# wolfcanli/ORB_SLAM2_Modification_with-point-and-line-feature

Measured on AMD Instinct MI355X. Metric: frames/sec (extract+match+pose) at 640x480; ATE RMSE vs ref, higher is better.
Workload: dtype u8

## Files before the change

### orb_slam2_modification_with-point-and-line-feature_amd/csrc/orb_extract.hip

```cpp
#include <hip/hip_runtime.h>
#include <algorithm>
#include <stdint.h>

#include <cstdlib>

#include "orb_geom.h"
#include "orbpl_math.h"
#include "orb_kernels.h"
#include "orbpl_runtime.h"

namespace orbpl {

#include "orb_pattern.inc"
__constant__ int c_pattern[1024];
__constant__ float4 c_pattern_f[256];

__device__ __forceinline__ int reflect101_dev(int p, int len) {
  if (p < 0) p = -p;
  if (p >= len) p = 2 * len - 2 - p;
  return p;
}

__host__ __device__ constexpr int fast_pstride(int win_w) { return (win_w + 7) & ~7; }
__host__ __device__ constexpr int fast_wave_words(int win_w, int win_h) {
  return win_h * (fast_pstride(win_w) / 2) + 4 * win_h;
}

typedef short fshort2 __attribute__((ext_vector_type(2)));
typedef unsigned short fushort2 __attribute__((ext_vector_type(2)));
typedef uint32_t fuint3 __attribute__((ext_vector_type(3)));
typedef fuint3 fuint3_a4 __attribute__((aligned(4)));

__device__ __forceinline__ uint32_t umul24(uint32_t a, uint32_t b) {
  return (uint32_t)(uint16_t)a * (uint32_t)(uint16_t)b;
}
template <uint32_t D>
__device__ __forceinline__ uint32_t div_c16(uint32_t i) {
  return umul24(i, (65536u + D - 1) / D) >> 16;
}
__device__ __forceinline__ int imul24(int a, int b) {
  return (int)(int16_t)a * (int)(int16_t)b;
}
__device__ __forceinline__ uint32_t ld_dw(const uint32_t* base, uint32_t dw) {
  return *reinterpret_cast<const uint32_t*>(reinterpret_cast<const char*>(base) + (dw << 2));
}
__device__ __forceinline__ void ld_dw3(const uint32_t* base, uint32_t dw, uint32_t* a, uint32_t* b,
                                       uint32_t* c) {
  const char* p = reinterpret_cast<const char*>(base) + (dw << 2);
  *a = *reinterpret_cast<const uint32_t*>(p);
  *b = *reinterpret_cast<const uint32_t*>(p + 4);
  *c = *reinterpret_cast<const uint32_t*>(p + 8);
}
__device__ __forceinline__ uint32_t ld_b4(const uint8_t* base, uint32_t off) {
  return *reinterpret_cast<const uint32_t*>(base + off);
}
__device__ __forceinline__ void st_b4(uint8_t* base, uint32_t off, uint32_t v) {
  *reinterpret_cast<uint32_t*>(base + off) = v;
}

__device__ __forceinline__ fshort2 as_s2(uint32_t v) { return __builtin_bit_cast(fshort2, v); }
__device__ __forceinline__ fushort2 as_u2(uint32_t v) { return __builtin_bit_cast(fushort2, v); }
__device__ __forceinline__ fshort2 pmin(fshort2 a, fshort2 b) { return __builtin_elementwise_min(a, b); }
__device__ __forceinline__ fshort2 pmax(fshort2 a, fshort2 b) { return __builtin_elementwise_max(a, b); }
__device__ __forceinline__ fushort2 pmaxu(fushort2 a, fushort2 b) { return __builtin_elementwise_max(a, b); }
__device__ __forceinline__ fushort2 pminu(fushort2 a, fushort2 b) { return __builtin_elementwise_min(a, b); }

__device__ __forceinline__ uint32_t ring_pair(const uint2* R, int dy, int dx) {
  const uint32_t j = (uint32_t)(3 + dx);
  return __builtin_amdgcn_perm(R[3 + dy].y, R[3 + dy].x, j | (0x0cu << 8) | ((j + 1) << 16) | (0x0cu << 24));
}

template <bool kMax>
__device__ __forceinline__ void fast_windows(const fushort2* p, fushort2* W) {
  auto op = [](fushort2 a, fushort2 b) { return kMax ? pmaxu(a, b) : pminu(a, b); };
  fushort2 s[2][4], pr[2][4];
#pragma unroll
  for (int h = 0; h < 2; h++) {
    const fushort2* d = p + 8 * h;
    const fushort2 q12 = op(d[1], d[2]), q34 = op(d[3], d[4]), q56 = op(d[5], d[6]);
    s[h][3] = d[7];
    s[h][2] = op(q56, d[7]);
    s[h][1] = op(q34, s[h][2]);
    s[h][0] = op(q12, s[h][1]);
    pr[h][0] = d[0];
    pr[h][1] = op(d[0], q12);
    pr[h][2] = op(pr[h][1], q34);
    pr[h][3] = op(pr[h][2], q56);
  }
#pragma unroll
  for (int i = 0; i < 4; i++) {
    W[i] = op(s[0][i], pr[1][i]);
    W[i + 4] = op(s[1][i], pr[0][i]);
  }
}

__device__ __forceinline__ fshort2 fast_m2_regs(const uint2* R) {
  const fushort2 v = as_u2(ring_pair(R, 0, 0));
  fushort2 p[16];
  p[0] = as_u2(ring_pair(R, 3, 0));
  p[1] = as_u2(ring_pair(R, 3, 1));
  p[2] = as_u2(ring_pair(R, 2, 2));
  p[3] = as_u2(ring_pair(R, 1, 3));
  p[4] = as_u2(ring_pair(R, 0, 3));
  p[5] = as_u2(ring_pair(R, -1, 3));
// ... 1148 lines not shown
        }
      }
    }
    __syncthreads();
    cur = nxt;
    size = newSize;
    if (size >= N || size == prevSize) {
      finish = true;
    } else if (!phase2 && size + nexp * 3 > N) {
      phase2 = true;
    }
  }
  lap(1);
  for (int i = t; i < size; i += NT) S.child[i] = 0;
  __syncthreads();
  for (int k = t; k < total; k += NT) {
    uint32_t c = K[k];
    int key = (cand_s(c) << 20) | (kMaxCandPerLevel - k);
    atomicMax(&S.child[kn_get(k)], key);
  }
  __syncthreads();
  const int cap = L.kp_cap;
  for (int i = t; i < size && i < cap; i += NT) {
    int k = kMaxCandPerLevel - (S.child[i] & kMaxCandPerLevel);
    out_list[i] = K[k];
  }
  if (t == 0) {
    if (size > cap) atomicOr(err_flag, 4);
    *out_count = size < cap ? size : cap;
  }
  lap(3);
  ot[5] = total;
  ot[6] = size;
  if (stamp)
    for (int k = 0; k < 8; k++) g_oct_prof[8 * level + k] = ot[k];
}

__device__ long long g_od_prof[8];

constexpr int kIcR = 15;
constexpr int kIcRowDw = 9;
constexpr int kIcDw = (2 * kIcR + 1) * kIcRowDw;
constexpr int kIcLoads = (kIcDw + 63) / 64;
constexpr int kBriefR = 18;
constexpr int kBriefRows = 2 * kBriefR + 1;
constexpr int kBriefRowDw = 10;
constexpr int kBriefDw = kBriefRows * kBriefRowDw;
constexpr int kBriefLoads = (kBriefDw + 63) / 64;

#ifndef ORBPL_OD_MINW
#define ORBPL_OD_MINW 1
#endif

__device__ __forceinline__ void ic_dword(uint32_t px, int u0, int um, int* s0, int* s1) {
  const int lo = min(max(-um - u0, 0), 4), hi = min(max(um - u0 + 1, 0), 4);
  const uint32_t m = hi > lo ? (0xFFFFFFFFu >> (8 * (4 - (hi - lo)))) << (8 * lo) : 0u;
  const uint32_t pm = px & m;
  const int a = (int)__builtin_amdgcn_udot4(pm, 0x01010101u, 0u, false);
  const int b = (int)__builtin_amdgcn_udot4(pm, 0x03020100u, 0u, false);
  *s0 += a;
  *s1 += imul24(u0, a) + b;
}
__global__ void __launch_bounds__(256, ORBPL_OD_MINW) k_orient_desc(const uint8_t* __restrict__ pyr,
                                                     const uint8_t* __restrict__ blur,
                                                     const OrbGeom* __restrict__ g,
                                                     const uint32_t* __restrict__ kp_list,
                                                     const int* __restrict__ kp_count,
                                                     orbpl_keypoint_dev* __restrict__ out_kps,
                                                     uint8_t* __restrict__ out_desc,
                                                     int kp_pitch, int* __restrict__ out_n,
                                                      int slot0, int slot1, int write_n) {
  __shared__ uint32_t s_patch[4][kBriefDw];
  const int wave = threadIdx.x >> 6, lane = threadIdx.x & 63;
  int bx, f;
  xcd_block(&bx, &f);
  const int slot = slot0 + bx * 4 + wave;
  if (slot >= slot1) return;
  const bool stamp = g_oct_prof_on && f == 0 && slot == 0 && lane == 0;
  long long dt[6] = {0, 0, 0, 0, 0, 0};
  long long d0 = stamp ? (long long)wall_clock64() : 0;
  auto lap = [&](int k) {
    if (stamp) {
      const long long d1 = (long long)wall_clock64();
      dt[k] = d1 - d0;
      d0 = d1;
    }
  };
  int level = 0;
  while (level + 1 < g->nlevels && slot >= g->lv[level + 1].kp_base) level++;
  const LevelGeom& L = g->lv[level];
  const int idx = slot - L.kp_base;
  const int* cnts = kp_count + (long long)f * g->nlevels;
  int offset = 0, total = 0;
  for (int l = 0; l < g->nlevels; l++) {
    int c = cnts[l];
    if (l < level) offset += c;
    total += c;
  }
  if (write_n && slot == slot0 && lane == 0) out_n[f] = total < kp_pitch ? total : kp_pitch;
  if (idx >= cnts[level]) return;
  const int opos = offset + idx;
  if (opos >= kp_pitch) return;
  lap(0);
  const uint32_t c = kp_list[(long long)f * g->kp_cap_total + slot];
  const int kx = cand_x(c) + kMinBorder, ky = cand_y(c) + kMinBorder;
  if (stamp) (void)__builtin_amdgcn_readfirstlane(kx);
  lap(1);
  const uint8_t* irow0 = pyr + (long long)f * g->pyr_bytes + content_off(L, kx - kIcR, ky - kIcR);
  const int io = (int)(reinterpret_cast<uintptr_t>(irow0) & 3);
  const uint32_t* irow = reinterpret_cast<const uint32_t*>(irow0 - io);
  const int ipdw = L.pitch >> 2;
  uint32_t iv[kIcLoads];
#pragma unroll
  for (int j = 0; j < kIcLoads; j++) {
    const int i = lane + 64 * j;
// ... 44 lines not shown
  cr_cos_sin(angle * factorPI, &a, &b);
  if (stamp) (void)__builtin_amdgcn_readfirstlane(__float_as_int(a + b));
  lap(3);
  uint32_t* patch = s_patch[wave];
#pragma unroll
  for (int j = 0; j < kBriefLoads; j++) {
    const int i = lane + 64 * j;
    if (i < kBriefDw) patch[i] = pv[j];
  }
  __builtin_amdgcn_wave_barrier();
  const uint8_t* bimg = reinterpret_cast<const uint8_t*>(patch) + kBriefR * 4 * kBriefRowDw +
                        (bx0 & 3) + kBriefR;
  const int step = 4 * kBriefRowDw;
  uint64_t words[4];
#pragma unroll
  for (int r = 0; r < 4; r++) {
    const int tst = r * 64 + lane;
    const int* p = &c_pattern[4 * tst];
    const float x1 = (float)p[0], y1 = (float)p[1], x2 = (float)p[2], y2 = (float)p[3];
    const int v1 = bimg[cv_round(x1 * b + y1 * a) * step + cv_round(x1 * a - y1 * b)];
    const int v2 = bimg[cv_round(x2 * b + y2 * a) * step + cv_round(x2 * a - y2 * b)];
    words[r] = __ballot(v1 < v2);
  }
  lap(4);
  uint8_t* d = out_desc + ((long long)f * kp_pitch + opos) * 32;
  if (lane < 4) {
    uint64_t w = lane == 0 ? words[0] : lane == 1 ? words[1] : lane == 2 ? words[2] : words[3];
    reinterpret_cast<uint64_t*>(d)[lane] = w;
  }
  if (lane == 0) {
    orbpl_keypoint_dev kp;
    float sx = (float)kx, sy = (float)ky;
    if (level != 0) {
      sx = sx * L.scale;
      sy = sy * L.scale;
    }
    kp.x = sx;
    kp.y = sy;
    kp.size = (float)L.scaled_patch;
    kp.angle = angle;
    kp.response = (float)cand_s(c);
    kp.octave = level;
    kp.class_id = -1;
    out_kps[(long long)f * kp_pitch + opos] = kp;
  }
  lap(5);
  if (stamp)
    for (int k = 0; k < 6; k++) g_od_prof[k] = dt[k];
}

#ifndef ORBPL_OD_PAIR
#define ORBPL_OD_PAIR 1
#endif
constexpr int kIcLoads2 = (kIcDw + 31) / 32;
constexpr int kBriefLoads2 = (kBriefDw + 31) / 32;
__global__ void __launch_bounds__(256, ORBPL_OD_MINW) k_orient_desc2(const uint8_t* __restrict__ pyr,
                                                      const uint8_t* __restrict__ blur,
                                                      const OrbGeom* __restrict__ g,
                                                      const uint32_t* __restrict__ kp_list,
                                                      const int* __restrict__ kp_count,
                                                      orbpl_keypoint_dev* __restrict__ out_kps,
                                                      uint8_t* __restrict__ out_desc,
                                                      int kp_pitch, int* __restrict__ out_n,
                                                      int slot0, int slot1, int write_n) {
  __shared__ uint32_t s_patch[8][kBriefDw];
  const int wave = threadIdx.x >> 6, lane = threadIdx.x & 63;
  const int half = lane >> 5, l32 = lane & 31;
  int bx, f;
  xcd_block(&bx, &f);
  const int slot = slot0 + bx * 8 + wave * 2 + half;
  const int nlev = g->nlevels;
  bool act = slot < slot1;
  int level = 0;
  if (act)
    while (level + 1 < nlev && slot >= g->lv[level + 1].kp_base) level++;
  const LevelGeom& L = g->lv[level];
  const int idx = slot - L.kp_base;
  const int* cnts = kp_count + (long long)f * nlev;
  int offset = 0, total = 0, mine = 0;
  for (int l = 0; l < nlev; l++) {
    const int c = cnts[l];
    if (l < level) offset += c;
    if (l == level) mine = c;
    total += c;
  }
  if (write_n && slot == slot0 && l32 == 0) out_n[f] = total < kp_pitch ? total : kp_pitch;
  act = act && idx < mine && offset + idx < kp_pitch;
  if (!__any(act)) return;
  const int opos = offset + idx;
  const uint32_t c = act ? kp_list[(long long)f * g->kp_cap_total + slot] : 0u;
  const int kx = act ? cand_x(c) + kMinBorder : kIcR + kBriefR,
            ky = act ? cand_y(c) + kMinBorder : kIcR + kBriefR;
  const uint32_t* fpyr = reinterpret_cast<const uint32_t*>(pyr + (long long)f * g->pyr_bytes);
  const int ioff = (int)content_off(L, kx - kIcR, ky - kIcR);
  const int io = ioff & 3;
  const uint32_t ibase = (uint32_t)ioff >> 2;
  const uint32_t ipdw = (uint32_t)L.pitch >> 2;
  uint32_t iv[kIcLoads2];
#pragma unroll
  for (int j = 0; j < kIcLoads2; j++) {
    const uint32_t i = (uint32_t)l32 + 32u * j;
    const uint32_t r = div_c16<kIcRowDw>(i), q = i - umul24(r, kIcRowDw);
    iv[j] = (act && i < (uint32_t)kIcDw) ? ld_dw(fpyr, ibase + umul24(r, ipdw) + q) : 0u;
  }
  const int bx0 = kx - kBriefR;
  const uint32_t* fblur = reinterpret_cast<const uint32_t*>(blur + (long long)f * g->blur_bytes);
  const uint32_t pdw = (uint32_t)L.bpitch >> 2;
  const uint32_t pbase =
      (uint32_t)((L.boff + (long long)(ky - kBriefR) * L.bpitch + (bx0 & ~3)) >> 2);
  uint32_t pv[kBriefLoads2];
#pragma unroll
  for (int j = 0; j < kBriefLoads2; j++) {
    const uint32_t i = (uint32_t)l32 + 32u * j;
    const uint32_t r = div_c16<kBriefRowDw>(i), q = i - umul24(r, kBriefRowDw);
    pv[j] = (act && i < (uint32_t)kBriefDw) ? ld_dw(fblur, pbase + umul24(r, pdw) + q) : 0u;
  }
  int m01 = 0, m10 = 0;
#pragma unroll
  for (int j = 0; j < kIcLoads2; j++) {
    const int i = l32 + 32 * j;
    const int r = (int)div_c16<kIcRowDw>((uint32_t)i), q = i - (int)umul24((uint32_t)r, kIcRowDw);
    const int v = r - kIcR;
    const int um = i < kIcDw ? g->umax[v < 0 ? -v : v] : -1;
    int s0 = 0;
    ic_dword(iv[j], 4 * q - io - kIcR, um, &s0, &m10);
    m01 += imul24(v, s0);
  }
#pragma unroll
  for (int o = 16; o >= 1; o >>= 1) {
    m10 += __shfl_xor(m10, o, 64);
    m01 += __shfl_xor(m01, o, 64);
  }
  const float angle = fast_atan2_deg((float)m01, (float)m10);
  const float factorPI = (float)(3.14159265358979323846 / 180.f);
  float a, b;
  cr_cos_sin(angle * factorPI, &a, &b);
  uint32_t* patch = s_patch[wave * 2 + half];
#pragma unroll
  for (int j = 0; j < kBriefLoads2; j++) {
    const int i = l32 + 32 * j;
    if (i < kBriefDw) patch[i] = pv[j];
  }
  __builtin_amdgcn_wave_barrier();
  const uint8_t* bimg = reinterpret_cast<const uint8_t*>(patch) + kBriefR * 4 * kBriefRowDw +
                        (bx0 & 3) + kBriefR;
  const int step = 4 * kBriefRowDw;
  uint32_t words[8];
#pragma unroll
  for (int r = 0; r < 8; r++) {
    const float4 P = c_pattern_f[r * 32 + l32];
    const float x1 = P.x, y1 = P.y, x2 = P.z, y2 = P.w;
    const float fs = (float)step;
    const int v1 = bimg[(int)(__builtin_rintf(x1 * b + y1 * a) * fs + __builtin_rintf(x1 * a - y1 * b))];
    const int v2 = bimg[(int)(__builtin_rintf(x2 * b + y2 * a) * fs + __builtin_rintf(x2 * a - y2 * b))];
    words[r] = (uint32_t)(__ballot(v1 < v2) >> (32 * half));
  }
  if (!act) return;
  uint8_t* d = out_desc + ((long long)f * kp_pitch + opos) * 32;
  if (l32 < 8) {
    uint32_t w = words[0];
#pragma unroll
    for (int r = 1; r < 8; r++) w = l32 == r ? words[r] : w;
    reinterpret_cast<uint32_t*>(d)[l32] = w;
  }
  if (l32 == 0) {
    orbpl_keypoint_dev kp;
    float sx = (float)kx, sy = (float)ky;
    if (level != 0) {
      sx = sx * L.scale;
      sy = sy * L.scale;
    }
    kp.x = sx;
    kp.y = sy;
    kp.size = (float)L.scaled_patch;
    kp.angle = angle;
    kp.response = (float)cand_s(c);
    kp.octave = level;
    kp.class_id = -1;
    out_kps[(long long)f * kp_pitch + opos] = kp;
  }
}

hipError_t upload_pattern(hipStream_t s) {
  static float pf[1024];
  static const bool filled = [] {
    for (int i = 0; i < 1024; i++) pf[i] = (float)bit_pattern_31_[i];
    return true;
  }();
  (void)filled;
  const hipError_t e = hipMemcpyToSymbolAsync(HIP_SYMBOL(c_pattern), bit_pattern_31_,
                                              sizeof(bit_pattern_31_), 0, hipMemcpyHostToDevice, s);
  if (e != hipSuccess) return e;
  return hipMemcpyToSymbolAsync(HIP_SYMBOL(c_pattern_f), pf, sizeof(pf), 0, hipMemcpyHostToDevice, s);
}
// ... 14 lines not shown
                    hipStream_t s) {
  hipLaunchKernelGGL(k_pyramid, dim3(nbands, batch), dim3(kPyrThreads), 0, s, img, stride,
                     frame_pitch, pyr, blur, dg, rs, bands, prof, l0, l1);
}

void launch_fast(const OrbGeom& hg, const OrbGeom* dg, const CellGeom* cells, const uint8_t* pyr,
                 uint32_t* cell_cands, int* cell_counts, int ini_th, int min_th, int batch,
                 int l0, int l1, hipStream_t s) {
  const size_t smem = 4 * 4 * (size_t)fast_wave_words(hg.fast_win_w, hg.fast_win_h);
  const int c0 = hg.lv[l0].cell_base;
  const int c1 = l1 < hg.nlevels ? hg.lv[l1].cell_base : hg.ncells_total;
  if (c1 <= c0) return;
  hipLaunchKernelGGL(k_fast_cells, dim3((c1 - c0 + 3) / 4, batch), dim3(256), smem, s, pyr, dg,
                     cells, cell_cands, cell_counts, ini_th, min_th, c0, c1);
}

void launch_octree(const OrbGeom& hg, const OrbGeom* dg, const uint32_t* cell_cands,
                   const int* cell_counts, uint32_t* kcand, int* knode, uint32_t* kp_list,
                   int* kp_count, int* err_flag, int batch, int l0, int l1, int wave_from,
                   hipStream_t s) {
  set_smem_attr((const void*)k_octree<1024, 256>, sizeof(OctShared<1024>));
  int cap = 0;
  for (int l = 0; l < hg.nlevels; l++) cap = std::max(cap, hg.lv[l].kp_cap);
  if (once_per_device((const void*)&g_oct_prof_on)) {
    const int on = getenv("ORBPL_OCT_PROFILE") ? 1 : 0;
    (void)hipMemcpyToSymbolAsync(HIP_SYMBOL(g_oct_prof_on), &on, sizeof(int), 0,
                                 hipMemcpyHostToDevice, s);
  }
  const bool one_wave = l0 >= (wave_from >= 0 ? wave_from : kOctWaveFrom);
#define ORBPL_OCT_LAUNCH(CAP)                                                                   \
  if (one_wave)                                                                                 \
    hipLaunchKernelGGL((k_octree<CAP, 64>), dim3(l1 - l0, batch), dim3(64),                    \
                       sizeof(OctShared<CAP, 2048>), s, dg, cell_cands, cell_counts, kcand,     \
                       knode,                                                                   \
                       kp_list, kp_count, err_flag, l0);                                        \
  else                                                                                          \
    hipLaunchKernelGGL((k_octree<CAP, 256>), dim3(l1 - l0, batch), dim3(256),                  \
                       sizeof(OctShared<CAP>), s, dg, cell_cands, cell_counts, kcand, knode,    \
                       kp_list, kp_count, err_flag, l0);
  if (cap <= 256) {
    ORBPL_OCT_LAUNCH(256)
  } else if (cap <= 512) {
    ORBPL_OCT_LAUNCH(512)
  } else {
    if (one_wave) set_smem_attr((const void*)k_octree<1024, 64>, sizeof(OctShared<1024, 2048>));
    ORBPL_OCT_LAUNCH(1024)
  }
#undef ORBPL_OCT_LAUNCH
}

void launch_orient_desc(const OrbGeom& hg, const OrbGeom* dg, const uint8_t* pyr,
                        const uint8_t* blur, const uint32_t* kp_list, const int* kp_count,
                        orbpl_keypoint_dev* out_kps, uint8_t* out_desc, int kp_pitch, int* out_n,
                        int batch, int l0, int l1, hipStream_t s) {
  const int s0 = hg.lv[l0].kp_base;
  const int s1 = l1 < hg.nlevels ? hg.lv[l1].kp_base : hg.kp_cap_total;
  const int wn = l1 == hg.nlevels ? 1 : 0;
  if (s1 <= s0) return;
  static const char* pe = getenv("ORBPL_OD_PAIR");
  static const bool pair = (pe ? atoi(pe) != 0 : ORBPL_OD_PAIR) && !getenv("ORBPL_OCT_PROFILE");
  if (pair)
    hipLaunchKernelGGL(k_orient_desc2, dim3((s1 - s0 + 7) / 8, batch), dim3(256), 0, s, pyr, blur,
                       dg, kp_list, kp_count, out_kps, out_desc, kp_pitch, out_n, s0, s1, wn);
  else
    hipLaunchKernelGGL(k_orient_desc, dim3((s1 - s0 + 3) / 4, batch), dim3(256), 0, s, pyr, blur,
                       dg, kp_list, kp_count, out_kps, out_desc, kp_pitch, out_n, s0, s1, wn);
}

}
```

### orb_slam2_modification_with-point-and-line-feature_amd/csrc/orb_geom.cpp

```cpp
#include <algorithm>
#include <cmath>
#include <vector>

#include "../../include/orbpl.h"
#include "orb_kernels.h"

namespace orbpl {

static int round_up(int v, int a) { return (v + a - 1) / a * a; }

int build_orb_geometry(int nfeatures, float scale_factor, int nlevels, int W, int H,
                       OrbHostGeom* out, const char** err) {
  *err = nullptr;
  if (nlevels < 1 || nlevels > kMaxLevels) { *err = "nlevels out of range [1,16]"; return ORBPL_ERR_ARG; }
  if (nfeatures < 1) { *err = "nfeatures must be >= 1"; return ORBPL_ERR_ARG; }
  if (!(scale_factor > 1.0f)) { *err = "scale_factor must be > 1"; return ORBPL_ERR_ARG; }
  if (W > 4000 || H > 4000) { *err = "image larger than 4000 px is not supported"; return ORBPL_ERR_ARG; }
  OrbHostGeom& G = *out;
  OrbGeom& g = G.g;
  g = OrbGeom{};
  g.nlevels = nlevels;
  g.W = W;
  g.H = H;
  const double sf = (double)scale_factor;
  G.scale.assign(nlevels, 1.0f);
  G.sigma2.assign(nlevels, 1.0f);
  for (int i = 1; i < nlevels; i++) {
    G.scale[i] = (float)(G.scale[i - 1] * sf);
    G.sigma2[i] = G.scale[i] * G.scale[i];
  }
  G.inv_scale.resize(nlevels);
  G.inv_sigma2.resize(nlevels);
  for (int i = 0; i < nlevels; i++) {
    G.inv_scale[i] = 1.0f / G.scale[i];
    G.inv_sigma2[i] = 1.0f / G.sigma2[i];
  }
  std::vector<int> nfeat(nlevels);
  {
    const float factor = (float)(1.0f / sf);
    float nd = nfeatures * (1 - factor) / (1 - (float)std::pow((double)factor, (double)nlevels));
    int sum = 0;
    for (int l = 0; l < nlevels - 1; l++) {
      nfeat[l] = (int)std::rint(nd);
      sum += nfeat[l];
      nd *= factor;
    }
    nfeat[nlevels - 1] = std::max(nfeatures - sum, 0);
  }
  {
    const int HP = 15;
    int v, v0;
    const int vmax = (int)std::floor(HP * std::sqrt(2.f) / 2 + 1);
    const int vmin = (int)std::ceil(HP * std::sqrt(2.f) / 2);
    const double hp2 = HP * HP;
    for (v = 0; v <= vmax; ++v) g.umax[v] = (int)std::rint(std::sqrt(hp2 - v * v));
    for (v = HP, v0 = 0; v >= vmin; --v) {
      while (g.umax[v0] == g.umax[v0 + 1]) ++v0;
      g.umax[v] = v0;
      ++v0;
    }
  }
  long long off = 0, boff = 0;
  int cell_total = 0, kp_total = 0;
  int max_slots = 1;
  G.cells.clear();
  G.rs.clear();
  std::vector<std::vector<CellGeom>> lvl_cells(nlevels);
  for (int l = 0; l < nlevels; l++) {
    LevelGeom& L = g.lv[l];
    L.w = (int)std::rint((float)W * G.inv_scale[l]);
    L.h = (int)std::rint((float)H * G.inv_scale[l]);
    if (L.w < 20 || L.h < 20) {
      *err = "a pyramid level is smaller than 20 px (image too small for nlevels/scale)";
      return ORBPL_ERR_ARG;
    }
    L.pw = L.w + 2 * kEdge;
    L.ph = L.h + 2 * kEdge;
    L.pitch = round_up(kLead + L.pw, 16);
    L.pyr_off = off;
    off += (long long)round_up(L.pitch * L.ph, 256);
    L.bpitch = round_up(L.w, 16);
    L.boff = boff;
    boff += (long long)round_up(L.bpitch * L.h, 256);
    L.scale = G.scale[l];
    L.nfeat = nfeat[l];
    L.scaled_patch = (int)(31 * G.scale[l]);
    const int minB = kMinBorder;
    const int maxBX = L.w - kEdge + 3, maxBY = L.h - kEdge + 3;
    L.max_border_x = maxBX;
    L.max_border_y = maxBY;
    const float width = (float)(maxBX - minB), height = (float)(maxBY - minB);
    const int nCols = (int)(width / 30.f), nRows = (int)(height / 30.f);
    L.ncols = nCols;
    L.nrows = nRows;
    L.wcell = nCols > 0 ? (int)std::ceil(width / nCols) : 0;
    L.hcell = nRows > 0 ? (int)std::ceil(height / nRows) : 0;
    L.ncells = nCols * nRows;
    L.cell_base = cell_total;
    for (int i = 0; i < nRows; i++) {
      const float iniY = (float)(minB + i * L.hcell);
      float maxY = iniY + L.hcell + 6;
      for (int j = 0; j < nCols; j++) {
        CellGeom c{};
        c.level = (int16_t)l;
        const float iniX = (float)(minB + j * L.wcell);
        float maxX = iniX + L.wcell + 6;
        bool skip = (iniY >= maxBY - 3) || (iniX >= maxBX - 6);
        if (!skip) {
          float my = maxY > maxBY ? (float)maxBY : maxY;
          float mx = maxX > maxBX ? (float)maxBX : maxX;
          c.x0 = (int16_t)iniX;
          c.y0 = (int16_t)iniY;
          c.x1 = (int16_t)mx;
// ... 111 lines not shown
```

### orb_slam2_modification_with-point-and-line-feature_amd/csrc/orb_geom.h

```cpp
#pragma once
#include <stdint.h>

namespace orbpl {

constexpr int kMaxLevels = 16;
constexpr int kEdge = 19;
constexpr int kMinBorder = 16;
constexpr int kLead = 13;
constexpr int kContent0 = kLead + 19;
constexpr int kOctMaxList = 1024;
constexpr int kMaxCandPerLevel = (1 << 20) - 1;

struct LevelGeom {
  int w, h;
  int pw, ph;
  int pitch;
  int pad0;
  long long pyr_off;
  float scale;
  int nfeat;
  int ncols, nrows;
  int wcell, hcell;
  int cell_base;
  int ncells;
  int max_border_x, max_border_y;
  int n_ini;
  float hx;
  int kp_cap;
  int kp_base;
  int cand_base;
  int cand_cap;
  int rs_off;
  int xmax;
  int scaled_patch;
  int pad2, pad3;
  int bpitch;
  int pad1;
  long long boff;
};

struct CellGeom {
  int16_t x0, y0, x1, y1;
  int16_t level, pad;
};

struct OrbGeom {
  int nlevels;
  int W, H;
  int ncells_total;
  int kp_cap_total;
  int cand_cap_total;
  int cell_slots;
  int fast_win_w;
  int fast_win_h;
  long long pyr_bytes;
  long long blur_bytes;
  int umax[16];
  LevelGeom lv[kMaxLevels];
};

#ifndef ORBPL_PYR_THREADS
#define ORBPL_PYR_THREADS 256
#endif
constexpr int kPyrThreads = ORBPL_PYR_THREADS;
constexpr int kPyrMaxBands = 8;
struct PyrBand {
  int na[kMaxLevels], nb[kMaxLevels];
  int oa[kMaxLevels], ob[kMaxLevels];
};
__host__ __device__ inline int pyr_band_base(int B) { return B - 1; }

__host__ __device__ inline long long content_off(const LevelGeom& L, int x, int y) {
  return L.pyr_off + (long long)(y + kEdge) * L.pitch + kContent0 + x;
}
__host__ __device__ inline long long padded_off(const LevelGeom& L, int px, int py) {
  return L.pyr_off + (long long)py * L.pitch + kLead + px;
}

__host__ __device__ inline uint32_t pack_cand(int x, int y, int s) {
  return (uint32_t)x | ((uint32_t)y << 12) | ((uint32_t)s << 24);
}
__host__ __device__ inline int cand_x(uint32_t c) { return (int)(c & 0xFFF); }
__host__ __device__ inline int cand_y(uint32_t c) { return (int)((c >> 12) & 0xFFF); }
__host__ __device__ inline int cand_s(uint32_t c) { return (int)(c >> 24); }

}
```

### orb_slam2_modification_with-point-and-line-feature_amd/csrc/orb_kernels.h

```cpp
#pragma once
#include <hip/hip_runtime.h>
#include <stdint.h>

#include <vector>

#include "orb_geom.h"

namespace orbpl {

struct orbpl_keypoint_dev {
  float x, y, size, angle, response;
  int octave, class_id;
};

hipError_t upload_pattern(hipStream_t s);
int read_octree_profile(long long* out128);
int read_od_profile(long long* out8);

void launch_pyramid(const OrbGeom& hg, const OrbGeom* dg, const uint8_t* img, int stride,
                    long long frame_pitch, uint8_t* pyr, uint8_t* blur, const int* rs,
                    const PyrBand* bands, int nbands, int batch, long long* prof, int l0, int l1,
                    hipStream_t s);
void launch_fast(const OrbGeom& hg, const OrbGeom* dg, const CellGeom* cells, const uint8_t* pyr,
                 uint32_t* cell_cands, int* cell_counts, int ini_th, int min_th, int batch,
                 int l0, int l1, hipStream_t s);
void launch_octree(const OrbGeom& hg, const OrbGeom* dg, const uint32_t* cell_cands,
                   const int* cell_counts, uint32_t* kcand, int* knode, uint32_t* kp_list,
                   int* kp_count, int* err_flag, int batch, int l0, int l1, int wave_from,
                   hipStream_t s);
void launch_orient_desc(const OrbGeom& hg, const OrbGeom* dg, const uint8_t* pyr,
                        const uint8_t* blur, const uint32_t* kp_list, const int* kp_count,
                        orbpl_keypoint_dev* out_kps, uint8_t* out_desc, int kp_pitch, int* out_n,
                        int batch, int l0, int l1, hipStream_t s);

struct OrbHostGeom {
  OrbGeom g;
  std::vector<CellGeom> cells;
  std::vector<int> rs;
  std::vector<PyrBand> bands;
  std::vector<float> scale, inv_scale, sigma2, inv_sigma2;
};
int build_orb_geometry(int nfeatures, float scale_factor, int nlevels, int W, int H,
                       OrbHostGeom* out, const char** err);

}
```

### orb_slam2_modification_with-point-and-line-feature_amd/csrc/orbpl_runtime.cpp

```cpp
#include <dirent.h>
#include <hip/hip_runtime.h>

#include <cstdio>
#include <cstdlib>
#include <cstring>
#include <unistd.h>
#include <mutex>
#include <map>
#include <set>
#include <cctype>
#include <string>
#include <utility>
#include <vector>

#include "../../include/orbpl.h"
#include "orb_kernels.h"
#include "host_stage.h"
#include "orbpl_runtime.h"

namespace orbpl {

int g_hw_queues = 4;
int g_runtime_started = 0;
int g_queues_set_by_lib = 0;
// ... 64 lines not shown
  static std::set<std::pair<const void*, int>> seen;
  int dev = 0;
  (void)hipGetDevice(&dev);
  std::lock_guard<std::mutex> lk(mu);
  return seen.insert({key, dev}).second;
}

void set_smem_attr(const void* fn, size_t bytes) {
  if (once_per_device(fn))
    (void)hipFuncSetAttribute(fn, hipFuncAttributeMaxDynamicSharedMemorySize, (int)bytes);
}

int device_cu_count() {
  static std::mutex mu;
  static std::map<int, int> cus;
  int dev = 0;
  (void)hipGetDevice(&dev);
  std::lock_guard<std::mutex> lk(mu);
  auto it = cus.find(dev);
  if (it != cus.end()) return it->second;
  int n = 0;
  if (hipDeviceGetAttribute(&n, hipDeviceAttributeMultiprocessorCount, dev) != hipSuccess || n <= 0)
    n = 256;
  cus[dev] = n;
  return n;
}

}

using namespace orbpl;

struct orbx_ctx {
  orbpl_orb_params params{};
  int device = 0;
  int max_batch = 0;
  OrbHostGeom hg;
  hipStream_t stream = nullptr;
  hipEvent_t ev[6] = {};
  hipStream_t fstream = nullptr;
  hipEvent_t ev_group[kMaxLevels] = {};
  hipEvent_t ev_fjoin = nullptr;
  hipEvent_t ev_kern[kKernelBrackets] = {};
  int ngroups = 1;
  int group_end[kMaxLevels] = {};
  bool timed = false;
  OrbGeom* d_geom = nullptr;
  CellGeom* d_cells = nullptr;
  int* d_rs = nullptr;
  PyrBand* d_bands = nullptr;
  long long* d_pyr_prof = nullptr;
  int pyr_bands = 0;
  int group_bands[kFastGroups] = {0, 0, 0, 0};
  int oct_wave_from = -1;
  uint8_t* d_in = nullptr;
  uint8_t* d_pyr = nullptr;
  uint8_t* d_blur = nullptr;
  uint32_t* d_cell_cands = nullptr;
  int* d_cell_counts = nullptr;
  uint32_t* d_kcand = nullptr;
  int* d_knode = nullptr;
  uint32_t* d_kp_list = nullptr;
  int* d_kp_count = nullptr;
  orbpl_keypoint_dev* d_out_kps = nullptr;
  uint8_t* d_out_desc = nullptr;
  int* d_out_n = nullptr;
  int* d_err = nullptr;
  int last_batch = 0;
};

extern "C" {

const char* orbpl_last_error(void) { return orbpl::g_last_error.c_str(); }

const char* orbpl_version(void) { return "orbpl gfx950 r4"; }

int orbpl_hw_queue_state(int* queues, int* runtime_started, int* set_by_library,
                         int* lsd_split_1024) {
  if (queues) *queues = orbpl::g_hw_queues;
  if (runtime_started) *runtime_started = orbpl::g_runtime_started;
  if (set_by_library) *set_by_library = orbpl::g_queues_set_by_lib;
  if (lsd_split_1024) *lsd_split_1024 = orbpl::lsd_split_decision(1024) ? 1 : 0;
  return ORBPL_OK;
}

int orbpl_device_count(int* n) {
  if (!n) return arg_fail("n is NULL");
  int c = 0;
  hipError_t e = hipGetDeviceCount(&c);
  if (e != hipSuccess) {
    *n = 0;
    hip_fail(e, "hipGetDeviceCount", __LINE__);
    return ORBPL_ERR_NODEVICE;
  }
  *n = c;
  return c > 0 ? ORBPL_OK : ORBPL_ERR_NODEVICE;
}

int orbpl_dev_malloc(int device, int64_t bytes, void** out) {
  if (!out || bytes < 0) return arg_fail("bad argument");
  HIP_CHECK(hipSetDevice(device));
  HIP_CHECK(hipMalloc(out, (size_t)(bytes > 0 ? bytes : 1)));
  return ORBPL_OK;
}

int orbpl_dev_free(int device, void* ptr) {
  HIP_CHECK(hipSetDevice(device));
// ... 140 lines not shown
    if (c->ngroups > 1) {
      CK(hipStreamCreateWithFlags(&c->fstream, hipStreamNonBlocking));
      for (int i = 0; i < c->ngroups; i++)
        CK(hipEventCreateWithFlags(&c->ev_group[i], hipEventDisableTiming));
      CK(hipEventCreateWithFlags(&c->ev_fjoin, hipEventDisableTiming));
    }
  }
  const size_t B = (size_t)max_batch;
  CK(hipMalloc(&c->d_geom, sizeof(OrbGeom)));
  CK(hipMalloc(&c->d_cells, sizeof(CellGeom) * std::max<size_t>(1, c->hg.cells.size())));
  CK(hipMalloc(&c->d_rs, sizeof(int) * c->hg.rs.size()));
  CK(hipMalloc(&c->d_bands, sizeof(PyrBand) * c->hg.bands.size()));
  CK(hipMalloc(&c->d_in, B * (size_t)width * height));
  CK(hipMalloc(&c->d_pyr, B * (size_t)g.pyr_bytes));
  CK(hipMalloc(&c->d_blur, B * (size_t)g.blur_bytes));
  CK(hipMalloc(&c->d_cell_cands, B * (size_t)std::max(1, g.ncells_total) * g.cell_slots * 4));
  CK(hipMalloc(&c->d_cell_counts, B * (size_t)std::max(1, g.ncells_total) * 4));
  CK(hipMalloc(&c->d_kcand, B * (size_t)std::max(1, g.cand_cap_total) * 4));
  CK(hipMalloc(&c->d_knode, B * (size_t)std::max(1, g.cand_cap_total) * 4));
  CK(hipMalloc(&c->d_kp_list, B * (size_t)g.kp_cap_total * 4));
  CK(hipMalloc(&c->d_kp_count, B * (size_t)g.nlevels * 4));
  CK(hipMalloc(&c->d_out_kps, B * (size_t)g.kp_cap_total * sizeof(orbpl_keypoint_dev)));
  CK(hipMalloc(&c->d_out_desc, B * (size_t)g.kp_cap_total * 32));
  CK(hipMalloc(&c->d_out_n, B * 4));
  CK(hipMalloc(&c->d_err, 4));
  CK(hipMemsetAsync(c->d_err, 0, 4, c->stream));
  CK(hipMemsetAsync(c->d_pyr, 0, B * (size_t)g.pyr_bytes, c->stream));
  CK(hipMemsetAsync(c->d_blur, 0, B * (size_t)g.blur_bytes, c->stream));
  CK(hipMemcpyAsync(c->d_geom, &g, sizeof(OrbGeom), hipMemcpyHostToDevice, c->stream));
  if (!c->hg.cells.empty())
    CK(hipMemcpyAsync(c->d_cells, c->hg.cells.data(), sizeof(CellGeom) * c->hg.cells.size(),
                      hipMemcpyHostToDevice, c->stream));
  CK(hipMemcpyAsync(c->d_rs, c->hg.rs.data(), sizeof(int) * c->hg.rs.size(), hipMemcpyHostToDevice,
                    c->stream));
  CK(hipMemcpyAsync(c->d_bands, c->hg.bands.data(), sizeof(PyrBand) * c->hg.bands.size(),
                    hipMemcpyHostToDevice, c->stream));
  if (const char* e = getenv("ORBPL_PYR_BANDS")) {
    const int b = atoi(e);
    if (b == 1 || b == 2 || b == 4 || b == 8) c->pyr_bands = b;
  }
  if (const char* e = getenv("ORBPL_PYR_GROUP_BANDS")) {
    int gi = 0;
    for (const char* q = e; *q && gi < kFastGroups;) {
      if (!isdigit((unsigned char)*q)) {
        q++;
        continue;
      }
      const int b = atoi(q);
      while (isdigit((unsigned char)*q)) q++;
      c->group_bands[gi++] = (b == 1 || b == 2 || b == 4 || b == 8) ? b : 0;
    }
  }
  if (const char* e = getenv("ORBPL_OCT_WAVE_FROM")) c->oct_wave_from = std::max(0, atoi(e));
  if (getenv("ORBPL_PYR_PROFILE")) {
    CK(hipMalloc(&c->d_pyr_prof, 8 * (1 + 4 * kMaxLevels)));
    CK(hipMemsetAsync(c->d_pyr_prof, 0, 8 * (1 + 4 * kMaxLevels), c->stream));
  }
  CK(upload_pattern(c->stream));
  CK(hipStreamSynchronize(c->stream));
#undef CK
  *out = c;
  return ORBPL_OK;
}

int orbx_debug_pyr_profile(orbx_ctx* c, long long* out, int cap, int* n) {
  if (!c || !out || !n) return arg_fail("bad argument");
  if (!c->d_pyr_prof) return arg_fail("ORBPL_PYR_PROFILE was not set when the context was created");
  HIP_CHECK(hipStreamSynchronize(c->stream));
  const int L = c->hg.g.nlevels;
  std::vector<long long> p(1 + 4 * kMaxLevels);
  HIP_CHECK(hipMemcpy(p.data(), c->d_pyr_prof, p.size() * 8, hipMemcpyDeviceToHost));
  *n = std::min(cap, 4 * L);
  for (int i = 0; i < *n; i++) out[i] = (p[i + 1] - p[i]) * 10;
  return ORBPL_OK;
}

int orbx_debug_octree_profile(orbx_ctx* c, long long* out128) {
  if (!c || !out128) return arg_fail("bad argument");
  HIP_CHECK(hipStreamSynchronize(c->stream));
  if (read_octree_profile(out128)) return arg_fail("octree profile unavailable");
  for (int l = 0; l < 16; l++)
    for (int k : {0, 1, 2, 3}) out128[8 * l + k] *= 10;
  long long od[6];
  if (read_od_profile(od) == 0)
    for (int k = 0; k < 6; k++) out128[120 + k] = od[k] * 10;
  return ORBPL_OK;
}

int orbx_destroy(orbx_ctx* c) {
  free_ctx(c);
  return ORBPL_OK;
}

int orbx_get_scale_info(const orbx_ctx* c, int* nlevels, float* scale, float* inv_scale,
                        float* sigma2, float* inv_sigma2) {
  if (!c) return arg_fail("NULL ctx");
  const int n = c->hg.g.nlevels;
  if (nlevels) *nlevels = n;
  for (int i = 0; i < n; i++) {
    if (scale) scale[i] = c->hg.scale[i];
    if (inv_scale) inv_scale[i] = c->hg.inv_scale[i];
    if (sigma2) sigma2[i] = c->hg.sigma2[i];
    if (inv_sigma2) inv_sigma2[i] = c->hg.inv_sigma2[i];
  }
  return ORBPL_OK;
}
// ... 32 lines not shown
namespace orbpl {
hipStream_t orbx_stream(orbx_ctx* c) { return c->stream; }

constexpr int kLevelPipeMinBatch = 64;

int orbx_run(orbx_ctx* c, const uint8_t* d_imgs, int batch, int stride, long long frame_pitch,
             orbpl_keypoint_dev* d_kps, uint8_t* d_desc, int kp_pitch, int* d_n,
             hipEvent_t* ext_events, hipEvent_t* ext_kernels) {
  const OrbGeom& g = c->hg.g;
  hipStream_t s = c->stream;
  c->timed = ext_events == nullptr;
  hipEvent_t* ev = ext_events ? ext_events : c->ev;
  hipEvent_t* evk = ext_kernels ? ext_kernels : (ext_events ? nullptr : c->ev_kern);
  HIP_CHECK(hipEventRecord(ev[0], s));
  int nb = c->pyr_bands;
  if (!nb) {
    nb = 1;
    while (nb < kPyrMaxBands && nb * batch < 1024) nb *= 2;
  }
  auto bracket = [&](int kind, int gi, int end, hipStream_t st) -> hipError_t {
    return evk ? hipEventRecord(evk[2 * (kind * kFastGroups + gi) + end], st) : hipSuccess;
  };
  const bool pipe = c->ngroups > 1 && batch >= kLevelPipeMinBatch;
  const int ngroups = pipe ? c->ngroups : 1;
  hipStream_t fs = pipe ? c->fstream : s;
  int l0 = 0;
  for (int gi = 0; gi < ngroups; gi++) {
    const int l1 = pipe ? c->group_end[gi] : g.nlevels;
    const int nbg = pipe && c->group_bands[gi] ? c->group_bands[gi] : nb;
    launch_pyramid(g, c->d_geom, d_imgs, stride, frame_pitch, c->d_pyr, c->d_blur, c->d_rs,
                   c->d_bands + pyr_band_base(nbg), nbg, batch, c->d_pyr_prof, l0, l1, s);
    if (pipe) {
      HIP_CHECK(hipEventRecord(c->ev_group[gi], s));
      HIP_CHECK(hipStreamWaitEvent(fs, c->ev_group[gi], 0));
    } else {
      HIP_CHECK(hipEventRecord(ev[1], s));
      HIP_CHECK(hipEventRecord(ev[2], s));
    }
    HIP_CHECK(bracket(0, gi, 0, fs));
    launch_fast(g, c->d_geom, c->d_cells, c->d_pyr, c->d_cell_cands, c->d_cell_counts,
                c->params.ini_th_fast, c->params.min_th_fast, batch, l0, l1, fs);
    HIP_CHECK(bracket(0, gi, 1, fs));
    if (!pipe) HIP_CHECK(hipEventRecord(ev[3], s));
    HIP_CHECK(bracket(1, gi, 0, fs));
    launch_octree(g, c->d_geom, c->d_cell_cands, c->d_cell_counts, c->d_kcand, c->d_knode,
                  c->d_kp_list, c->d_kp_count, c->d_err, batch, l0, l1, c->oct_wave_from,
                  fs);
    HIP_CHECK(bracket(1, gi, 1, fs));
    if (!pipe) HIP_CHECK(hipEventRecord(ev[4], s));
    l0 = l1;
  }
  HIP_CHECK(bracket(2, 0, 0, fs));
  launch_orient_desc(g, c->d_geom, c->d_pyr, c->d_blur, c->d_kp_list, c->d_kp_count, d_kps, d_desc,
                     kp_pitch, d_n, batch, 0, g.nlevels, fs);
  HIP_CHECK(bracket(2, 0, 1, fs));
  for (int kind = 0; kind < 3; kind++)
    for (int gi = kind == 2 ? 1 : ngroups; gi < kFastGroups; gi++) {
      HIP_CHECK(bracket(kind, gi, 0, fs));
      HIP_CHECK(bracket(kind, gi, 1, fs));
    }
  if (pipe) {
    HIP_CHECK(hipEventRecord(ev[1], s));
    HIP_CHECK(hipEventRecord(ev[2], s));
    HIP_CHECK(hipEventRecord(c->ev_fjoin, fs));
    HIP_CHECK(hipStreamWaitEvent(s, c->ev_fjoin, 0));
    HIP_CHECK(hipEventRecord(ev[3], s));
    HIP_CHECK(hipEventRecord(ev[4], s));
  }
  HIP_CHECK(hipEventRecord(ev[5], s));
  HIP_CHECK(hipGetLastError());
  c->last_batch = batch;
  return ORBPL_OK;
}
}

extern "C" {

int orbx_synchronize(orbx_ctx* c) {
  if (!c) return arg_fail("NULL ctx");
  HIP_CHECK(hipSetDevice(c->device));
  HIP_CHECK(hipStreamSynchronize(c->stream));
  int flag = 0;
  HIP_CHECK(hipMemcpy(&flag, c->d_err, 4, hipMemcpyDeviceToHost));
  if (flag) {
    HIP_CHECK(hipMemset(c->d_err, 0, 4));
    char buf[128];
    snprintf(buf, sizeof(buf), "kernel capacity overflow (flags 0x%x)", flag);
    orbpl::g_last_error = buf;
    return ORBPL_ERR_OVERFLOW;
  }
  return ORBPL_OK;
}

int orbx_extract(orbx_ctx* c, const uint8_t* img, int width, int height, int stride,
                 orbpl_keypoint* kps, uint8_t* desc, int cap, int* n) {
  if (!c || !n) return arg_fail("NULL argument");
  *n = 0;
  if (!img || width <= 0 || height <= 0) return ORBPL_OK;
  if (width != c->hg.g.W || height != c->hg.g.H)
    return arg_fail("image size differs from the size given to orbx_create");
  if (stride < width) return arg_fail("stride < width");
  HIP_CHECK(hipSetDevice(c->device));
  const OrbGeom& g = c->hg.g;
  HIP_CHECK(hipMemcpy2DAsync(c->d_in, width, img, stride, width, height, hipMemcpyHostToDevice,
                             c->stream));
  int rc = orbx_run(c, c->d_in, 1, width, (long long)width * height, c->d_out_kps, c->d_out_desc,
                    g.kp_cap_total, c->d_out_n);
// ... 130 lines not shown
```

Measured before the change: 130,400.

## Restructure orient/descriptor patch loads into row-strided lanes with precomputed IC masks

In the paired orient/descriptor kernel, each lane now owns a fixed column dword and a row phase. It loads every third row by adding a constant stride, which removes the per-load divide and modulo address math. The intensity-centroid circular masks are precomputed on the host into the geometry struct per alignment offset, and the moments are accumulated with dot4 instructions instead of recomputing umax masks on the device. The cross-lane reduction uses ds_swizzle instead of shfl_xor, and the pair-mode env lookup moves into the context. The cost is a larger geometry struct and extra per-lane mask loads from global memory.

Result: no change. 131,000, median of 3 (+0.5%).

```diff
diff --git a/orb_slam2_modification_with-point-and-line-feature_amd/csrc/orb_extract.hip b/orb_slam2_modification_with-point-and-line-feature_amd/csrc/orb_extract.hip
--- a/orb_slam2_modification_with-point-and-line-feature_amd/csrc/orb_extract.hip
+++ b/orb_slam2_modification_with-point-and-line-feature_amd/csrc/orb_extract.hip
@@ -40,9 +40,6 @@
 }
 __device__ __forceinline__ int imul24(int a, int b) {
   return (int)(int16_t)a * (int)(int16_t)b;
-}
-__device__ __forceinline__ uint32_t ld_dw(const uint32_t* base, uint32_t dw) {
-  return *reinterpret_cast<const uint32_t*>(reinterpret_cast<const char*>(base) + (dw << 2));
 }
 __device__ __forceinline__ void ld_dw3(const uint32_t* base, uint32_t dw, uint32_t* a, uint32_t* b,
                                        uint32_t* c) {
@@ -50,6 +47,10 @@
   *a = *reinterpret_cast<const uint32_t*>(p);
   *b = *reinterpret_cast<const uint32_t*>(p + 4);
   *c = *reinterpret_cast<const uint32_t*>(p + 8);
+}
+template <int O>
+__device__ __forceinline__ int swz_xor32(int v) {
+  return __builtin_amdgcn_ds_swizzle(v, (O << 10) | 0x1f);
 }
 __device__ __forceinline__ uint32_t ld_b4(const uint8_t* base, uint32_t off) {
   return *reinterpret_cast<const uint32_t*>(base + off);
@@ -1304,15 +1305,6 @@
 #define ORBPL_OD_MINW 1
 #endif
 
-__device__ __forceinline__ void ic_dword(uint32_t px, int u0, int um, int* s0, int* s1) {
-  const int lo = min(max(-um - u0, 0), 4), hi = min(max(um - u0 + 1, 0), 4);
-  const uint32_t m = hi > lo ? (0xFFFFFFFFu >> (8 * (4 - (hi - lo)))) << (8 * lo) : 0u;
-  const uint32_t pm = px & m;
-  const int a = (int)__builtin_amdgcn_udot4(pm, 0x01010101u, 0u, false);
-  const int b = (int)__builtin_amdgcn_udot4(pm, 0x03020100u, 0u, false);
-  *s0 += a;
-  *s1 += imul24(u0, a) + b;
-}
 __global__ void __launch_bounds__(256, ORBPL_OD_MINW) k_orient_desc(const uint8_t* __restrict__ pyr,
                                                      const uint8_t* __restrict__ blur,
                                                      const OrbGeom* __restrict__ g,
@@ -1463,8 +1455,14 @@
 #ifndef ORBPL_OD_PAIR
 #define ORBPL_OD_PAIR 1
 #endif
-constexpr int kIcLoads2 = (kIcDw + 31) / 32;
-constexpr int kBriefLoads2 = (kBriefDw + 31) / 32;
+constexpr int kOdRows = kIcMapRows;
+constexpr int kIcLanes2 = kIcMapLanes;
+constexpr int kIcLoads2 = kIcMapLoads;
+constexpr int kBriefLanes2 = kOdRows * kBriefRowDw;
+constexpr int kBriefLoads2 = (kBriefRows + kOdRows - 1) / kOdRows;
+static_assert(kIcLanes2 == kOdRows * kIcRowDw && (kIcLoads2 - 1) * kOdRows == 2 * kIcR,
+              "the last IC load holds row 30 alone");
+static_assert((kBriefLoads2 - 1) * kOdRows == kBriefRows - 1, "the last BRIEF load holds row 36 alone");
 __global__ void __launch_bounds__(256, ORBPL_OD_MINW) k_orient_desc2(const uint8_t* __restrict__ pyr,
                                                       const uint8_t* __restrict__ blur,
                                                       const OrbGeom* __restrict__ g,
@@ -1502,55 +1500,73 @@
   const uint32_t c = act ? kp_list[(long long)f * g->kp_cap_total + slot] : 0u;
   const int kx = act ? cand_x(c) + kMinBorder : kIcR + kBriefR,
             ky = act ? cand_y(c) + kMinBorder : kIcR + kBriefR;
-  const uint32_t* fpyr = reinterpret_cast<const uint32_t*>(pyr + (long long)f * g->pyr_bytes);
-  const int ioff = (int)content_off(L, kx - kIcR, ky - kIcR);
-  const int io = ioff & 3;
-  const uint32_t ibase = (uint32_t)ioff >> 2;
-  const uint32_t ipdw = (uint32_t)L.pitch >> 2;
+  const uint8_t* fpyr = pyr + (long long)f * g->pyr_bytes;
+  const uint32_t ipitch = (uint32_t)L.pitch;
+  const uint32_t ioff = (uint32_t)L.pyr_off + umul24((uint32_t)(ky - kIcR + kEdge), ipitch) +
+                        (uint32_t)(kContent0 + kx - kIcR);
+  const int io = (int)(ioff & 3u);
+  const uint32_t ir0 = div_c16<kIcRowDw>((uint32_t)l32), iq = (uint32_t)l32 - ir0 * kIcRowDw;
+  const bool ic_lane = act && l32 < kIcLanes2;
+  const bool ic_last = ic_lane && l32 < kIcRowDw;
+  const uint32_t istep = kOdRows * ipitch;
   uint32_t iv[kIcLoads2];
-#pragma unroll
-  for (int j = 0; j < kIcLoads2; j++) {
-    const uint32_t i = (uint32_t)l32 + 32u * j;
-    const uint32_t r = div_c16<kIcRowDw>(i), q = i - umul24(r, kIcRowDw);
-    iv[j] = (act && i < (uint32_t)kIcDw) ? ld_dw(fpyr, ibase + umul24(r, ipdw) + q) : 0u;
+  uint4 mk[kIcMapPitch / 4];
+  if (ic_lane) {
+    uint32_t o = (ioff & ~3u) + umul24(ir0, ipitch) + 4u * iq;
+#pragma unroll
+    for (int j = 0; j < kIcLoads2 - 1; j++, o += istep) iv[j] = ld_b4(fpyr, o);
+    if (ic_last) iv[kIcLoads2 - 1] = ld_b4(fpyr, o);
+#pragma unroll
+    for (int k = 0; k < kIcMapPitch / 4; k++)
+      mk[k] = *reinterpret_cast<const uint4*>(g->ic_mask[io][k][l32]);
   }
   const int bx0 = kx - kBriefR;
-  const uint32_t* fblur = reinterpret_cast<const uint32_t*>(blur + (long long)f * g->blur_bytes);
-  const uint32_t pdw = (uint32_t)L.bpitch >> 2;
-  const uint32_t pbase =
-      (uint32_t)((L.boff + (long long)(ky - kBriefR) * L.bpitch + (bx0 & ~3)) >> 2);
+  const uint8_t* fblur = blur + (long long)f * g->blur_bytes;
+  const uint32_t bpitch = (uint32_t)L.bpitch;
+  const uint32_t br0 = div_c16<kBriefRowDw>((uint32_t)l32), bq = (uint32_t)l32 - br0 * kBriefRowDw;
+  const bool br_lane = act && l32 < kBriefLanes2;
+  const bool br_last = br_lane && l32 < kBriefRowDw;
+  const uint32_t pstep = kOdRows * bpitch;
   uint32_t pv[kBriefLoads2];
-#pragma unroll
-  for (int j = 0; j < kBriefLoads2; j++) {
-    const uint32_t i = (uint32_t)l32 + 32u * j;
-    const uint32_t r = div_c16<kBriefRowDw>(i), q = i - umul24(r, kBriefRowDw);
-    pv[j] = (act && i < (uint32_t)kBriefDw) ? ld_dw(fblur, pbase + umul24(r, pdw) + q) : 0u;
+  if (br_lane) {
+    uint32_t o = (uint32_t)L.boff + umul24((uint32_t)(ky - kBriefR) + br0, bpitch) +
+                 (uint32_t)(bx0 & ~3) + 4u * bq;
+#pragma unroll
+    for (int j = 0; j < kBriefLoads2 - 1; j++, o += pstep) pv[j] = ld_b4(fblur, o);
+    if (br_last) pv[kBriefLoads2 - 1] = ld_b4(fblur, o);
   }
   int m01 = 0, m10 = 0;
-#pragma unroll
-  for (int j = 0; j < kIcLoads2; j++) {
-    const int i = l32 + 32 * j;
-    const int r = (int)div_c16<kIcRowDw>((uint32_t)i), q = i - (int)umul24((uint32_t)r, kIcRowDw);
-    const int v = r - kIcR;
-    const int um = i < kIcDw ? g->umax[v < 0 ? -v : v] : -1;
-    int s0 = 0;
-    ic_dword(iv[j], 4 * q - io - kIcR, um, &s0, &m10);
-    m01 += imul24(v, s0);
-  }
-#pragma unroll
-  for (int o = 16; o >= 1; o >>= 1) {
-    m10 += __shfl_xor(m10, o, 64);
-    m01 += __shfl_xor(m01, o, 64);
-  }
+  if (ic_lane) {
+    const uint32_t wp = __builtin_amdgcn_perm(4u * iq, 4u * iq, 0u) + 0x03020100u;
+    uint32_t s0 = 0, s1 = 0, sp = 0;
+    auto dword = [&](int j) {
+      const uint4 m4 = mk[j >> 2];
+      const uint32_t m = (j & 3) == 0 ? m4.x : (j & 3) == 1 ? m4.y : (j & 3) == 2 ? m4.z : m4.w;
+      const uint32_t pm = iv[j] & m;
+      s0 = __builtin_amdgcn_udot4(pm, 0x01010101u, s0, false);
+      if (j) s1 = __builtin_amdgcn_udot4(pm, 0x01010101u * (uint32_t)j, s1, false);
+      sp = __builtin_amdgcn_udot4(pm, wp, sp, false);
+    };
+#pragma unroll
+    for (int j = 0; j < kIcLoads2 - 1; j++) dword(j);
+    if (ic_last) dword(kIcLoads2 - 1);
+    m01 = imul24((int)ir0 - kIcR, (int)s0) + kOdRows * (int)s1;
+    m10 = (int)sp - imul24(io + kIcR, (int)s0);
+  }
+  m10 += swz_xor32<16>(m10); m01 += swz_xor32<16>(m01);
+  m10 += swz_xor32<8>(m10);  m01 += swz_xor32<8>(m01);
+  m10 += swz_xor32<4>(m10);  m01 += swz_xor32<4>(m01);
+  m10 += swz_xor32<2>(m10);  m01 += swz_xor32<2>(m01);
+  m10 += swz_xor32<1>(m10);  m01 += swz_xor32<1>(m01);
   const float angle = fast_atan2_deg((float)m01, (float)m10);
   const float factorPI = (float)(3.14159265358979323846 / 180.f);
   float a, b;
   cr_cos_sin(angle * factorPI, &a, &b);
   uint32_t* patch = s_patch[wave * 2 + half];
-#pragma unroll
-  for (int j = 0; j < kBriefLoads2; j++) {
-    const int i = l32 + 32 * j;
-    if (i < kBriefDw) patch[i] = pv[j];
+  if (br_lane) {
+#pragma unroll
+    for (int j = 0; j < kBriefLoads2 - 1; j++) patch[l32 + kBriefLanes2 * j] = pv[j];
+    if (br_last) patch[l32 + kBriefLanes2 * (kBriefLoads2 - 1)] = pv[kBriefLoads2 - 1];
   }
   __builtin_amdgcn_wave_barrier();
   const uint8_t* bimg = reinterpret_cast<const uint8_t*>(patch) + kBriefR * 4 * kBriefRowDw +
@@ -1671,13 +1687,13 @@
 void launch_orient_desc(const OrbGeom& hg, const OrbGeom* dg, const uint8_t* pyr,
                         const uint8_t* blur, const uint32_t* kp_list, const int* kp_count,
                         orbpl_keypoint_dev* out_kps, uint8_t* out_desc, int kp_pitch, int* out_n,
-                        int batch, int l0, int l1, hipStream_t s) {
+                        int batch, int l0, int l1, int od_pair, hipStream_t s) {
   const int s0 = hg.lv[l0].kp_base;
   const int s1 = l1 < hg.nlevels ? hg.lv[l1].kp_base : hg.kp_cap_total;
   const int wn = l1 == hg.nlevels ? 1 : 0;
   if (s1 <= s0) return;
-  static const char* pe = getenv("ORBPL_OD_PAIR");
-  static const bool pair = (pe ? atoi(pe) != 0 : ORBPL_OD_PAIR) && !getenv("ORBPL_OCT_PROFILE");
+  static const bool prof = getenv("ORBPL_OCT_PROFILE") != nullptr;
+  const bool pair = (od_pair >= 0 ? od_pair != 0 : ORBPL_OD_PAIR != 0) && !prof;
   if (pair)
     hipLaunchKernelGGL(k_orient_desc2, dim3((s1 - s0 + 7) / 8, batch), dim3(256), 0, s, pyr, blur,
                        dg, kp_list, kp_count, out_kps, out_desc, kp_pitch, out_n, s0, s1, wn);
diff --git a/orb_slam2_modification_with-point-and-line-feature_amd/csrc/orb_geom.cpp b/orb_slam2_modification_with-point-and-line-feature_amd/csrc/orb_geom.cpp
--- a/orb_slam2_modification_with-point-and-line-feature_amd/csrc/orb_geom.cpp
+++ b/orb_slam2_modification_with-point-and-line-feature_amd/csrc/orb_geom.cpp
@@ -1,5 +1,6 @@
 #include <algorithm>
 #include <cmath>
+#include <cstdlib>
 #include <vector>
 
 #include "../../include/orbpl.h"
@@ -59,6 +60,17 @@
       g.umax[v] = v0;
       ++v0;
     }
+    for (int io = 0; io < 4; io++)
+      for (int lane = 0; lane < kIcMapLanes; lane++)
+        for (int j = 0; j < kIcMapLoads; j++) {
+          const int q = lane % 9, row = lane / 9 + kIcMapRows * j;
+          if (row > 2 * HP) continue;
+          const int um = g.umax[std::abs(row - HP)];
+          uint32_t m = 0;
+          for (int bq = 0; bq < 4; bq++)
+            if (std::abs(4 * q + bq - io - HP) <= um) m |= 0xFFu << (8 * bq);
+          g.ic_mask[io][j / 4][lane][j % 4] = m;
+        }
   }
   long long off = 0, boff = 0;
   int cell_total = 0, kp_total = 0;
diff --git a/orb_slam2_modification_with-point-and-line-feature_amd/csrc/orb_geom.h b/orb_slam2_modification_with-point-and-line-feature_amd/csrc/orb_geom.h
--- a/orb_slam2_modification_with-point-and-line-feature_amd/csrc/orb_geom.h
+++ b/orb_slam2_modification_with-point-and-line-feature_amd/csrc/orb_geom.h
@@ -44,6 +44,11 @@
   int16_t level, pad;
 };
 
+constexpr int kIcMapRows = 3;
+constexpr int kIcMapLanes = kIcMapRows * 9;
+constexpr int kIcMapLoads = 11;
+constexpr int kIcMapPitch = 12;
+
 struct OrbGeom {
   int nlevels;
   int W, H;
@@ -57,6 +62,7 @@
   long long blur_bytes;
   int umax[16];
   LevelGeom lv[kMaxLevels];
+  alignas(16) uint32_t ic_mask[4][kIcMapPitch / 4][kIcMapLanes][4];
 };
 
 #ifndef ORBPL_PYR_THREADS
diff --git a/orb_slam2_modification_with-point-and-line-feature_amd/csrc/orb_kernels.h b/orb_slam2_modification_with-point-and-line-feature_amd/csrc/orb_kernels.h
--- a/orb_slam2_modification_with-point-and-line-feature_amd/csrc/orb_kernels.h
+++ b/orb_slam2_modification_with-point-and-line-feature_amd/csrc/orb_kernels.h
@@ -31,7 +31,7 @@
 void launch_orient_desc(const OrbGeom& hg, const OrbGeom* dg, const uint8_t* pyr,
                         const uint8_t* blur, const uint32_t* kp_list, const int* kp_count,
                         orbpl_keypoint_dev* out_kps, uint8_t* out_desc, int kp_pitch, int* out_n,
-                        int batch, int l0, int l1, hipStream_t s);
+                        int batch, int l0, int l1, int od_pair, hipStream_t s);
 
 struct OrbHostGeom {
   OrbGeom g;
diff --git a/orb_slam2_modification_with-point-and-line-feature_amd/csrc/orbpl_runtime.cpp b/orb_slam2_modification_with-point-and-line-feature_amd/csrc/orbpl_runtime.cpp
--- a/orb_slam2_modification_with-point-and-line-feature_amd/csrc/orbpl_runtime.cpp
+++ b/orb_slam2_modification_with-point-and-line-feature_amd/csrc/orbpl_runtime.cpp
@@ -140,6 +140,7 @@
   int pyr_bands = 0;
   int group_bands[kFastGroups] = {0, 0, 0, 0};
   int oct_wave_from = -1;
+  int od_pair = -1;
   uint8_t* d_in = nullptr;
   uint8_t* d_pyr = nullptr;
   uint8_t* d_blur = nullptr;
@@ -386,6 +387,7 @@
     }
   }
   if (const char* e = getenv("ORBPL_OCT_WAVE_FROM")) c->oct_wave_from = std::max(0, atoi(e));
+  if (const char* e = getenv("ORBPL_OD_PAIR")) c->od_pair = atoi(e) != 0 ? 1 : 0;
   if (getenv("ORBPL_PYR_PROFILE")) {
     CK(hipMalloc(&c->d_pyr_prof, 8 * (1 + 4 * kMaxLevels)));
     CK(hipMemsetAsync(c->d_pyr_prof, 0, 8 * (1 + 4 * kMaxLevels), c->stream));
@@ -524,7 +526,7 @@
   }
   HIP_CHECK(bracket(2, 0, 0, fs));
   launch_orient_desc(g, c->d_geom, c->d_pyr, c->d_blur, c->d_kp_list, c->d_kp_count, d_kps, d_desc,
-                     kp_pitch, d_n, batch, 0, g.nlevels, fs);
+                     kp_pitch, d_n, batch, 0, g.nlevels, c->od_pair, fs);
   HIP_CHECK(bracket(2, 0, 1, fs));
   for (int kind = 0; kind < 3; kind++)
     for (int gi = kind == 2 ? 1 : ngroups; gi < kFastGroups; gi++) {
```
